# rishikksh20/FastSpeech2

Hardware: NVIDIA H100
Metric: mel-frames/sec (batched inference) (higher is better)
Workload: dtype 3xf16

## Files before the change

fastspeech2_b200/csrc/gemm_tc.cu:

```cuda
#include <stdlib.h>

#include "tc_common.cuh"

namespace fs2 {
namespace {
using namespace tc;

constexpr int BM = 128;
constexpr int BK = 32;
constexpr int A_BYTES = BM * BK * 4;
constexpr int THREADS = 384;
constexpr int PRODUCER_REGS = 40, CONSUMER_REGS = 232;
constexpr int RING_BUDGET = 227 * 1024 - 1024  - 256 ;

struct TcParams {
  int L, tiles_per_utt;
  int m_tiles, n_tiles;
  int B, full, gn, upt, full_tiles;
  int K, taps, pad;
  const float* bias; const float* resid; int ldr; int act;
  float* out; int ldo;
  float a_inv; const float* w_inv;
  __half* outp; __half* outp_lo; int ldo_p;
  float* vt_out; __half* vtp; __half* vtp_lo; int vt_col0, vt_dk, vt_heads, vt_lpad, vt_L;
  const int64_t* lens;
};

template <int BN, bool PRECISE, bool HALF = false>
struct Cfg {
  static constexpr int B_BYTES = BN * BK * 4;
  static constexpr int STAGE_BYTES = (PRECISE ? 2 : 1) * (A_BYTES + B_BYTES);
  static_assert(!PRECISE || HALF, "the error-compensated family is 3xF16");
  static constexpr int STAGES = (RING_BUDGET / STAGE_BYTES) > 8 ? 8 : (RING_BUDGET / STAGE_BYTES);
  static constexpr size_t SMEM = (size_t)STAGES * STAGE_BYTES + 1024 + 256;
  static constexpr int BKE = HALF ? 2 * BK : BK;
  static constexpr int A_LO = A_BYTES;
  static constexpr int B_HI = PRECISE ? 2 * A_BYTES : A_BYTES;
  static constexpr int B_LO = B_HI + B_BYTES;
  static constexpr uint32_t TX_BYTES = (PRECISE ? 2 : 1) * (A_BYTES + B_BYTES);
  static_assert(BN % 16 == 0 && BN >= 16 && BN <= 128, "tile width: sums of wgmma N = 128 / 64 / 16");
  static_assert(B_BYTES % 1024 == 0, "B stage must keep 1024-byte alignment");
  static_assert(STAGES >= 2, "resources");
};

template <int BN, bool HALF, int C0 = 0>
__device__ __forceinline__ void mma_tile(float* d, uint64_t a, uint64_t b, uint32_t acc) {
  if constexpr (BN - C0 >= 128) {
    if constexpr (HALF) wgmma_f16_n128(d + C0 / 2, a, b + (C0 * 128 >> 4), acc); else wgmma_tf32_n128(d + C0 / 2, a, b + (C0 * 128 >> 4), acc);
    mma_tile<BN, HALF, C0 + 128>(d, a, b, acc);
  } else if constexpr (BN - C0 >= 64) {
    if constexpr (HALF) wgmma_f16_n64(d + C0 / 2, a, b + (C0 * 128 >> 4), acc); else wgmma_tf32_n64(d + C0 / 2, a, b + (C0 * 128 >> 4), acc);
    mma_tile<BN, HALF, C0 + 64>(d, a, b, acc);
  } else if constexpr (BN - C0 >= 16) {
    if constexpr (HALF) wgmma_f16_n16(d + C0 / 2, a, b + (C0 * 128 >> 4), acc); else wgmma_tf32_n16(d + C0 / 2, a, b + (C0 * 128 >> 4), acc);
    mma_tile<BN, HALF, C0 + 16>(d, a, b, acc);
  }
}

template <int BN, bool PRECISE, bool HALF>
__global__ void __launch_bounds__(THREADS, 1)
tap_gemm_tc_kernel(const __grid_constant__ CUtensorMap tmap_a, const __grid_constant__ CUtensorMap tmap_b,
                   const __grid_constant__ CUtensorMap tmap_b_lo, const __grid_constant__ CUtensorMap tmap_a16, TcParams p) {
  using C = Cfg<BN, PRECISE, HALF>;
  extern __shared__ uint8_t smem_raw[];
  uint8_t* tiles = smem_raw + ((1024u - (smem_u32(smem_raw) & 1023u)) & 1023u);
  uint64_t* full_bar = reinterpret_cast<uint64_t*>(tiles + (size_t)C::STAGES * C::STAGE_BYTES);
  uint64_t* empty_bar = full_bar + C::STAGES;

  const int warp = uniform_warp_idx(), lane = threadIdx.x & 31;
  const int kchunks = (p.K + C::BKE - 1) / C::BKE;
  const int steps = p.taps * kchunks;
  const int total_tiles = p.m_tiles * p.n_tiles;

  uint64_t* order_bar = empty_bar + C::STAGES;

  if (threadIdx.x == 0) {
    for (int s = 0; s < C::STAGES; ++s) { mbar_init(&full_bar[s], 1); mbar_init(&empty_bar[s], 4); }
    mbar_init(&order_bar[0], 4); mbar_init(&order_bar[1], 4);
    asm volatile("fence.mbarrier_init.release.cluster;" ::: "memory");
  }
  __syncthreads();
  pdl_wait();

  auto tile_coords = [&](int tile, int& n0, int& b, int& t0, int& packed) -> bool {
    const int mt = tile / p.n_tiles;
    n0 = (tile - mt * p.n_tiles) * BN;
    packed = -1;
    if (p.tiles_per_utt == 0) { b = 0; t0 = mt * BM; }
    else if (mt < p.full_tiles) { b = mt / p.full; t0 = (mt - b * p.full) * BM; }
    else { packed = mt - p.full_tiles; b = packed * p.upt; t0 = p.full * BM; }
    return packed < 0 && p.lens != nullptr && t0 >= p.lens[b];
  };

  if (warp < 4) {
    setmaxnreg_dec<PRODUCER_REGS>();
    if (warp != 0) { pdl_trigger(); return; }
    const uint32_t tiles_addr = smem_u32(tiles), full_addr = smem_u32(full_bar);
    int n = 0;
    for (int tile = blockIdx.x; tile < total_tiles; tile += gridDim.x) {
      int n0, b, t0, packed;
      if (tile_coords(tile, n0, b, t0, packed)) continue;
      int j = 0, kc = 0;
      for (int s = 0; s < steps; ++s, ++n) {
        const int slot = n % C::STAGES, round = n / C::STAGES;
        const int k0 = kc * C::BKE, row = t0 + j - p.pad;
        const uint32_t st = tiles_addr + (uint32_t)slot * C::STAGE_BYTES, fb = full_addr + (uint32_t)slot * 8u;
        pin_before(st, fb, k0, row);
        mbar_wait(&empty_bar[slot], (round & 1) ^ 1);
        mbar_expect_tx_elect(fb, C::TX_BYTES);
        if (packed < 0) {
          tma_load_3d_elect(st, &tmap_a, fb, k0, row, b);
          if (PRECISE) tma_load_3d_elect(st + C::A_LO, &tmap_a, fb, k0, row, b + p.B);
        } else {
          for (int g = 0; g < 8; ++g) {
            const int u = g / p.gn, gi = g - u * p.gn;
            const bool real = u < p.upt && b + u < p.B;
            const int oob = PRECISE ? 2 * p.B : p.B;
            tma_load_3d_elect(st + g * (16 * 128), &tmap_a16, fb, k0, row + gi * 16, real ? b + u : oob);
            if (PRECISE) tma_load_3d_elect(st + C::A_LO + g * (16 * 128), &tmap_a16, fb, k0, row + gi * 16, real ? b + u + p.B : oob);
          }
        }
        tma_load_3d_elect(st + C::B_HI, &tmap_b, fb, k0, n0, j);
        if (PRECISE) tma_load_3d_elect(st + C::B_LO, &tmap_b_lo, fb, k0, n0, j);
        if (++kc == kchunks) { kc = 0; ++j; }
      }
    }
  } else {
    setmaxnreg_inc<CONSUMER_REGS>();
    const int cg = (warp >> 2) - 1, wq = warp & 3;
    const int r_lo = 16 * wq + (lane >> 2);
    const int act = p.act, ldr = p.ldr, ldo = p.ldo;
    const float* __restrict__ resid = p.resid; float* __restrict__ out = p.out;
    const bool has_res = resid != nullptr;
    const float oscale = p.a_inv * (p.w_inv ? __ldg(p.w_inv) : 1.0f);
    float d[BN];
    int n = 0;
    int k = 0;
    for (int tile = blockIdx.x; tile < total_tiles; tile += gridDim.x, ++k) {
      int n0, b, t0, packed;
      const int tile_steps = tile_coords(tile, n0, b, t0, packed) ? 0 : steps;
      if ((k & 1) != cg) { n += tile_steps; continue; }
      long m[4]; bool row_ok[4], row_zero[4];
#pragma unroll
      for (int i = 0; i < 4; ++i) {
        const int row = 64 * (i >> 1) + r_lo + 8 * (i & 1);
        int bb = b, t = t0 + row;
        bool ok = t < p.L;
        if (packed >= 0) {
          const int g = row >> 4, u = g / p.gn, gi = g - u * p.gn;
          bb += u;
          t = t0 + gi * 16 + (row & 15);
          ok = u < p.upt && bb < p.B && t < p.L;
        }
        m[i] = (long)bb * p.L + t; row_ok[i] = ok;
        row_zero[i] = ok && p.lens != nullptr && t >= p.lens[bb];
        if (has_res && ok) prefetch_l2(resid + m[i] * ldr + n0);
      }
      if (k > 0) mbar_wait(&order_bar[cg], ((k - 1) >> 1) & 1);
      int prev = -1;
      for (int s = 0; s < tile_steps; ++s, ++n) {
        const int slot = n % C::STAGES, round = n / C::STAGES;
        const uint32_t base = smem_u32(tiles + (size_t)slot * C::STAGE_BYTES);
        const uint64_t a_hi = make_sw128_kmajor_desc(base), b_hi = make_sw128_kmajor_desc(base + C::B_HI);
        const uint64_t a_lo = make_sw128_kmajor_desc(base + C::A_LO), b_lo = make_sw128_kmajor_desc(base + C::B_LO);
        constexpr uint64_t HALF_A = (A_BYTES / 2) >> 4;
        mbar_wait(&full_bar[slot], round & 1);
        wgmma_fence();
#pragma unroll
        for (int kk = 0; kk < 4; ++kk) {
#pragma unroll
          for (int hf = 0; hf < 2; ++hf) {
            float* dh = d + hf * (BN / 2);
            if (PRECISE) {
              mma_tile<BN, true>(dh, a_lo + hf * HALF_A + 2 * kk, b_hi + 2 * kk, (s | kk) != 0);
              mma_tile<BN, true>(dh, a_hi + hf * HALF_A + 2 * kk, b_lo + 2 * kk, 1);
              mma_tile<BN, true>(dh, a_hi + hf * HALF_A + 2 * kk, b_hi + 2 * kk, 1);
            } else {
              mma_tile<BN, HALF>(dh, a_hi + hf * HALF_A + 2 * kk, b_hi + 2 * kk, (s | kk) != 0);
            }
          }
        }
        wgmma_commit();
        wgmma_wait<1>();
        pin_regs<BN>(d);
        if (prev >= 0) { __syncwarp(); if (lane == 0) mbar_arrive(&empty_bar[prev]); }
        prev = slot;
      }
      __syncwarp();
      if (lane == 0) mbar_arrive(&order_bar[cg ^ 1]);
      wgmma_wait<0>();
      pin_regs<BN>(d);
      if (prev >= 0) { __syncwarp(); if (lane == 0) mbar_arrive(&empty_bar[prev]); }
      if (tile_steps == 0) {
#pragma unroll
        for (int i = 0; i < BN; ++i) d[i] = 0.f;
      }

      const bool to_vt = (p.vt_out != nullptr || p.vtp != nullptr) && n0 >= p.vt_col0;
#pragma unroll
      for (int i = 0; i < 4; ++i) {
        if (!row_ok[i] || (to_vt && row_zero[i])) continue;
        const long mm = m[i];
        float* dr = d + (i >> 1) * (BN / 2) + 2 * (i & 1);
#pragma unroll
        for (int jj = 0; jj < BN / 8; ++jj) {
          const int col = n0 + 8 * jj + 2 * (lane & 3);
          float v0 = dr[4 * jj], v1 = dr[4 * jj + 1];
          const float b0 = p.bias ? __ldg(p.bias + col) : 0.f, b1 = p.bias ? __ldg(p.bias + col + 1) : 0.f;
          v0 = fmaf(v0, oscale, b0); v1 = fmaf(v1, oscale, b1);
          if (!to_vt) {
            if (act == ACT_RELU) { v0 = fmaxf(v0, 0.f); v1 = fmaxf(v1, 0.f); }
            else if (act == ACT_TANH) { v0 = tanhf(v0); v1 = tanhf(v1); }
            if (has_res) {
              const float2 r = __ldg(reinterpret_cast<const float2*>(resid + mm * ldr + col));
              v0 += r.x; v1 += r.y;
            }
            if (row_zero[i]) { v0 = 0.f; v1 = 0.f; }
          }
          dr[4 * jj] = v0; dr[4 * jj + 1] = v1;
        }
        if (to_vt) {
          const long ub = mm / p.vt_L;
          const long orow = ub * p.vt_heads * p.vt_dk * (long)p.vt_lpad + (mm - ub * p.vt_L);
#pragma unroll
          for (int jj = 0; jj < BN / 8; ++jj) {
            const int col = n0 + 8 * jj + 2 * (lane & 3);
            const float v0 = dr[4 * jj], v1 = dr[4 * jj + 1];
            const long o = orow + (long)(col - p.vt_col0) * p.vt_lpad;
            if (p.vt_out != nullptr) {
              p.vt_out[o] = v0; p.vt_out[o + p.vt_lpad] = v1;
            } else {
              uint32_t hi, lo;
              split_pair(v0, v1, hi, lo);
              const __half2 h2 = *reinterpret_cast<const __half2*>(&hi), l2 = *reinterpret_cast<const __half2*>(&lo);
              p.vtp[o] = __low2half(h2); p.vtp[o + p.vt_lpad] = __high2half(h2);
              if (p.vtp_lo != nullptr) { p.vtp_lo[o] = __low2half(l2); p.vtp_lo[o + p.vt_lpad] = __high2half(l2); }
            }
          }
          continue;
        }
#pragma unroll
        for (int jj = 0; jj < BN / 8; ++jj) {
          const int col = n0 + 8 * jj + 2 * (lane & 3);
          const float v0 = dr[4 * jj], v1 = dr[4 * jj + 1];
          if (HALF && p.outp != nullptr) {
            const long off = mm * p.ldo_p + col;
            if (p.outp_lo != nullptr) {
              uint32_t hi, lo;
              split_pair(v0, v1, hi, lo);
              *reinterpret_cast<uint32_t*>(p.outp + off) = hi;
              *reinterpret_cast<uint32_t*>(p.outp_lo + off) = lo;
            } else {
              *reinterpret_cast<uint32_t*>(p.outp + off) = hi_pair(v0, v1);
            }
          }
          if (out != nullptr) *reinterpret_cast<float2*>(out + mm * ldo + col) = make_float2(v0, v1);
        }
      }
    }
  }
  pdl_trigger();
}

__global__ void split_rows_f16_kernel(const float* __restrict__ x, int ldx, long rows, int K, __half* __restrict__ S) {
  pdl_trigger(); pdl_wait();
  const int kq = K >> 2;
  const long quads = rows * kq;
  __half* __restrict__ lo_plane = S + rows * K;
  for (long i = (long)blockIdx.x * blockDim.x + threadIdx.x; i < quads; i += (long)gridDim.x * blockDim.x) {
    const long r = i / kq;
    const int c = (int)(i - r * kq) * 4;
    const float4 v = *reinterpret_cast<const float4*>(x + r * ldx + c);
    uint2 hv, lv;
    split_pair(v.x, v.y, hv.x, lv.x);
    split_pair(v.z, v.w, hv.y, lv.y);
    *reinterpret_cast<uint2*>(S + r * K + c) = hv;
    *reinterpret_cast<uint2*>(lo_plane + r * K + c) = lv;
  }
}

template <int BN, bool PRECISE, bool HALF = false>
int launch(const TapGemm& g, cudaStream_t st) {
  using C = Cfg<BN, PRECISE, HALF>;
  static unsigned long long configured = 0;
  int rc;
  if ((rc = ensure_smem_attr(tap_gemm_tc_kernel<BN, PRECISE, HALF>, C::SMEM, &configured))) return rc;
  TcParams p;
  p.K = g.K; p.taps = g.taps; p.pad = (g.taps - 1) / 2;
  p.bias = g.bias; p.resid = g.resid; p.ldr = g.ldr; p.act = g.act; p.out = g.out; p.ldo = g.ldo;
  const long rows = (long)g.B * g.L;
  p.a_inv = HALF ? g.a_inv : 1.0f; p.w_inv = HALF ? g.w_inv : nullptr;
  p.outp = HALF ? g.outp : nullptr; p.ldo_p = g.ldo_p;
  p.outp_lo = (HALF && g.outp && g.outp_lo) ? g.outp + rows * g.ldo_p : nullptr;
  p.vt_out = HALF ? nullptr : g.vt_out; p.vtp = HALF ? g.vtp : nullptr;
  p.vtp_lo = (HALF && g.vtp && g.outp_lo) ? g.vtp + (long)g.B * g.vt_heads * g.vt_dk * g.vt_lpad : nullptr;
  p.vt_col0 = g.vt_col0; p.vt_dk = g.vt_dk; p.vt_heads = g.vt_heads; p.vt_lpad = g.vt_lpad; p.vt_L = g.L;
  p.lens = g.lens;
  CUtensorMap ma, mb, mb_lo, ma16;
  const int esz = HALF ? 2 : 4;
  constexpr int planes = HALF && PRECISE ? 2 : 1;
  const void* xa = HALF ? (const void*)g.xp : (const void*)g.x;
  const uint64_t row_bytes = HALF ? (uint64_t)g.K * 2 : (uint64_t)g.ldx * 4;
  if (g.taps == 1 && g.lens == nullptr) {
    const uint64_t M = (uint64_t)g.B * g.L;
    p.L = (int)M; p.tiles_per_utt = 0;
    p.m_tiles = (int)((M + BM - 1) / BM);
    p.B = 1; p.full = 0; p.gn = 1; p.upt = 1; p.full_tiles = 0;
    if ((rc = make_map(&ma, xa, g.K, M, planes, row_bytes, row_bytes * M, BM, HALF))) return rc;
    ma16 = ma;
  } else {
    p.L = g.L; p.tiles_per_utt = (g.L + BM - 1) / BM;
    p.B = g.B; p.full = g.L / BM;
    int tail = g.L % BM;
    p.gn = tail ? (tail + 15) / 16 : 1;
    p.upt = tail ? 8 / p.gn : 1;
    if (tail && p.upt == 1) { p.full += 1; tail = 0; p.gn = 1; }
    p.full_tiles = p.full * g.B;
    p.m_tiles = p.full_tiles + (tail ? (g.B + p.upt - 1) / p.upt : 0);
    if ((rc = make_map(&ma, xa, g.K, g.L, (uint64_t)g.B * planes, row_bytes, row_bytes * g.L, BM, HALF))) return rc;
    if ((rc = make_map(&ma16, xa, g.K, g.L, (uint64_t)g.B * planes, row_bytes, row_bytes * g.L, 16, HALF))) return rc;
  }
  p.n_tiles = g.N / BN;
  const void* w_hi = HALF ? (const void*)g.w_hi : (const void*)g.w;
  if ((rc = make_map(&mb, w_hi, g.K, g.N, g.taps, (uint64_t)g.K * esz, (uint64_t)g.K * esz * g.N, BN, HALF))) return rc;
  if ((rc = make_map(&mb_lo, PRECISE ? (const void*)g.w_lo : w_hi, g.K, g.N, g.taps, (uint64_t)g.K * esz, (uint64_t)g.K * esz * g.N, BN, HALF))) return rc;
  const int total = p.m_tiles * p.n_tiles;
  const int grid = total < sm_count_current() ? total : sm_count_current();
  FS2_CUDA_CHECK(launch_pdl(tap_gemm_tc_kernel<BN, PRECISE, HALF>, dim3(grid), dim3(THREADS), C::SMEM, st, ma, mb, mb_lo, ma16, p));
  FS2_LAUNCH_CHECK();
  return FS2_OK;
}

int tile_width(int N) { return N % 128 == 0 ? 128 : N % 80 == 0 ? 80 : N % 64 == 0 ? 64 : N % 32 == 0 ? 32 : 16; }

template <bool PRECISE, bool HALF>
int launch_any(const TapGemm& g, cudaStream_t st) {
  switch (tile_width(g.N)) {
    case 128: return launch<128, PRECISE, HALF>(g, st);
    case 80: return launch<80, PRECISE, HALF>(g, st);
    case 64: return launch<64, PRECISE, HALF>(g, st);
    case 32: return launch<32, PRECISE, HALF>(g, st);
    default: return launch<16, PRECISE, HALF>(g, st);
  }
}

int check_output(const TapGemm& g, const char* who) {
  FS2_REQUIRE((g.taps & 1) == 1, "%s: taps must be odd", who);
  FS2_REQUIRE(g.N % 16 == 0, "%s: N (%d) must be a multiple of 16", who, g.N);
  FS2_REQUIRE(!g.resid || g.ldr % 4 == 0, "%s: row strides must be 16-byte multiples", who);
  FS2_REQUIRE(!g.out || (g.ldo % 8 == 0 && (reinterpret_cast<uintptr_t>(g.out) & 31) == 0), "%s: output rows must be 32-byte aligned", who);
  return FS2_OK;
}
int check_common(const TapGemm& g, const char* who) {
  FS2_REQUIRE(g.K % 4 == 0, "%s: K (%d) must be a multiple of 4", who, g.K);
  FS2_REQUIRE(g.ldx % 4 == 0, "%s: row strides must be 16-byte multiples", who);
  FS2_REQUIRE((reinterpret_cast<uintptr_t>(g.x) & 15) == 0 && (reinterpret_cast<uintptr_t>(g.w) & 15) == 0 && g.out != nullptr,
              "%s: operands must be 16-byte aligned", who);
  return check_output(g, who);
}

}

int tap_gemm_tf32(const TapGemm& g, cudaStream_t st) {
  int rc = check_common(g, "tap_gemm_tf32");
  if (rc) return rc;
  FS2_REQUIRE(!g.vt_out || g.vt_col0 % tile_width(g.N) == 0, "tap_gemm_tf32: the transposed V third must start at a tile boundary");
  if ((long)g.B * g.L == 0) return FS2_OK;
  return launch_any<false, false>(g, st);
}

int tap_gemm_planes(const TapGemm& g, cudaStream_t st) {
  const char* who = g.precise ? "tap_gemm_planes(3xF16)" : "tap_gemm_planes(f16)";
  FS2_REQUIRE(g.xp && g.w_hi && (!g.precise || g.w_lo) && (g.out || g.outp || g.vtp), "%s: operand planes / an output missing", who);
  FS2_REQUIRE(g.K % 8 == 0, "%s: K (%d) must be a multiple of 8 (16-byte plane rows)", who, g.K);
  FS2_REQUIRE((reinterpret_cast<uintptr_t>(g.xp) & 15) == 0 && (reinterpret_cast<uintptr_t>(g.w_hi) & 15) == 0, "%s: operands must be 16-byte aligned", who);
  FS2_REQUIRE(!g.outp || (g.ldo_p % 16 == 0 && (reinterpret_cast<uintptr_t>(g.outp) & 31) == 0 && (((long)g.B * g.L * g.ldo_p) % 16) == 0),
              "%s: output plane rows must be 32-byte aligned", who);
  {
    const int bn = tile_width(g.N);
    FS2_REQUIRE(!g.vtp || (g.vt_lpad % 8 == 0 && g.N % bn == 0 && g.vt_col0 % bn == 0 && g.vt_dk % 32 == 0),
                "%s: transposed V planes need a 16-byte row pitch and tile-aligned thirds", who);
  }
  int rc = check_output(g, who);
  if (rc) return rc;
  if ((long)g.B * g.L == 0) return FS2_OK;
  return g.precise ? launch_any<true, true>(g, st) : launch_any<false, true>(g, st);
}

int split_rows(const float* x, int ldx, long rows, int K, __half* planes, cudaStream_t st) {
  if (rows == 0) return FS2_OK;
  FS2_REQUIRE(K % 4 == 0 && ldx % 4 == 0, "split_rows: K and the row stride must be multiples of 4");
  const long quads = rows * (K / 4);
  long blocks = (quads + 255) / 256;
  FS2_CUDA_CHECK(launch_pdl(split_rows_f16_kernel, dim3((unsigned)(blocks > 132 * 16 ? 132 * 16 : blocks)), dim3(256), 0, st, x, ldx, rows, K, planes));
  FS2_LAUNCH_CHECK();
  return FS2_OK;
}

namespace {
__global__ void split_f16_kernel(const float* __restrict__ src, __half* __restrict__ hi, __half* __restrict__ lo, long n,
                                 const float* __restrict__ scale) {
  const float s = scale ? __ldg(scale) : 1.0f;
  for (long i = (long)blockIdx.x * blockDim.x + threadIdx.x; i < n; i += (long)gridDim.x * blockDim.x) {
    const float x = fminf(fmaxf(src[i] * s, -65504.f), 65504.f);
    const __half h = __float2half_rn(x);
    hi[i] = h; lo[i] = __float2half_rn(x - __half2float(h));
  }
}
__global__ void weight_scale_kernel(const float* __restrict__ w, long n, float* __restrict__ scale, float* __restrict__ inv) {
  __shared__ float red[32];
  float m = 0.f;
  for (long i = threadIdx.x; i < n; i += blockDim.x) m = fmaxf(m, fabsf(w[i]));
  m = warp_max(m);
  if ((threadIdx.x & 31) == 0) red[threadIdx.x >> 5] = m;
  __syncthreads();
  if (threadIdx.x < 32) {
    m = threadIdx.x < (blockDim.x >> 5) ? red[threadIdx.x] : 0.f;
    m = warp_max(m);
    if (threadIdx.x == 0) {
      int k = 0;
      if (m > 0.f && isfinite(m)) {
        int e;
        frexpf(m, &e);
        k = 14 - e;
        k = k > 60 ? 60 : (k < -60 ? -60 : k);
      }
      scale[0] = ldexpf(1.0f, k); inv[0] = ldexpf(1.0f, -k);
    }
  }
}
}

namespace {
__global__ void planes_to_rows_kernel(const __half* __restrict__ planes, long n, float* __restrict__ out) {
  for (long i = (long)blockIdx.x * blockDim.x + threadIdx.x; i < n; i += (long)gridDim.x * blockDim.x)
    out[i] = (__half2float(planes[i]) + __half2float(planes[n + i])) * kPlaneInv;
}
}

int planes_to_rows(const __half* planes, long n, float* out, cudaStream_t st) {
  if (n == 0) return FS2_OK;
  long blocks = (n + 255) / 256;
  planes_to_rows_kernel<<<(int)(blocks > 1184 ? 1184 : blocks), 256, 0, st>>>(planes, n, out);
  FS2_LAUNCH_CHECK();
  return FS2_OK;
}

int split_f16(const float* src, __half* hi, __half* lo, long n, const float* scale, cudaStream_t st) {
  if (n == 0) return FS2_OK;
  long blocks = (n + 255) / 256;
  split_f16_kernel<<<(int)(blocks > 1184 ? 1184 : blocks), 256, 0, st>>>(src, hi, lo, n, scale);
  FS2_LAUNCH_CHECK();
  return FS2_OK;
}

int weight_scale(const float* w, long n, float* scale, float* inv, cudaStream_t st) {
  weight_scale_kernel<<<1, 1024, 0, st>>>(w, n, scale, inv);
  FS2_LAUNCH_CHECK();
  return FS2_OK;
}

}
```

Baseline: 2.927 million.

## Load conv halo A tile once per k-chunk and reuse across taps

Splits the shared-memory ring into separate A and B rings. For multi-tap convolutions the A tile is loaded once per k-chunk as a halo box of BM+taps-1 rows and reused across all taps by shifting the descriptor base by one row per tap; previously each tap reloaded a full A tile. Ring depths are computed at launch time and the loop order becomes k-chunk outer, taps inner. This cuts A-operand TMA traffic by roughly the tap count, at the cost of more complex barrier bookkeeping. The one-row descriptor offset relies on the swizzle layout lining up, which is a correctness risk.

```diff
diff --git a/fastspeech2_b200/csrc/gemm_tc.cu b/fastspeech2_b200/csrc/gemm_tc.cu
--- a/fastspeech2_b200/csrc/gemm_tc.cu
+++ b/fastspeech2_b200/csrc/gemm_tc.cu
@@ -11,13 +11,18 @@
 constexpr int A_BYTES = BM * BK * 4;
 constexpr int THREADS = 384;
 constexpr int PRODUCER_REGS = 40, CONSUMER_REGS = 232;
-constexpr int RING_BUDGET = 227 * 1024 - 1024  - 256 ;
+constexpr int MAX_DEPTH = 8;
+constexpr int BAR_BYTES = (4 * MAX_DEPTH + 2) * 8;
+constexpr int SMEM_MAX = 227 * 1024;
+constexpr int RING_BUDGET = SMEM_MAX - 1024  - BAR_BYTES;
+constexpr int MAX_BOX_ROWS = 256;
 
 struct TcParams {
   int L, tiles_per_utt;
   int m_tiles, n_tiles;
   int B, full, gn, upt, full_tiles;
   int K, taps, pad;
+  int a_rows, a_plane, a_slot, a_depth, b_depth;
   const float* bias; const float* resid; int ldr; int act;
   float* out; int ldo;
   float a_inv; const float* w_inv;
@@ -28,20 +33,30 @@
 
 template <int BN, bool PRECISE, bool HALF = false>
 struct Cfg {
+  static constexpr int PLANES = PRECISE ? 2 : 1;
   static constexpr int B_BYTES = BN * BK * 4;
-  static constexpr int STAGE_BYTES = (PRECISE ? 2 : 1) * (A_BYTES + B_BYTES);
+  static constexpr int B_SLOT = PLANES * B_BYTES;
   static_assert(!PRECISE || HALF, "the error-compensated family is 3xF16");
-  static constexpr int STAGES = (RING_BUDGET / STAGE_BYTES) > 8 ? 8 : (RING_BUDGET / STAGE_BYTES);
-  static constexpr size_t SMEM = (size_t)STAGES * STAGE_BYTES + 1024 + 256;
   static constexpr int BKE = HALF ? 2 * BK : BK;
-  static constexpr int A_LO = A_BYTES;
-  static constexpr int B_HI = PRECISE ? 2 * A_BYTES : A_BYTES;
-  static constexpr int B_LO = B_HI + B_BYTES;
-  static constexpr uint32_t TX_BYTES = (PRECISE ? 2 : 1) * (A_BYTES + B_BYTES);
   static_assert(BN % 16 == 0 && BN >= 16 && BN <= 128, "tile width: sums of wgmma N = 128 / 64 / 16");
-  static_assert(B_BYTES % 1024 == 0, "B stage must keep 1024-byte alignment");
-  static_assert(STAGES >= 2, "resources");
+  static_assert(B_BYTES % 1024 == 0, "B slot must keep 1024-byte alignment");
 };
+
+template <int BN, bool PRECISE, bool HALF>
+bool ring_layout(int taps, TcParams& p) {
+  using C = Cfg<BN, PRECISE, HALF>;
+  p.a_rows = BM + taps - 1;
+  p.a_plane = (p.a_rows * 128 + 1023) / 1024 * 1024;
+  p.a_slot = C::PLANES * p.a_plane;
+  auto cap = [](int d) { return d > MAX_DEPTH ? MAX_DEPTH : d; };
+  if (taps == 1) {
+    p.a_depth = p.b_depth = cap(RING_BUDGET / (p.a_slot + C::B_SLOT));
+  } else {
+    p.b_depth = cap((RING_BUDGET - 2 * p.a_slot) / C::B_SLOT);
+    p.a_depth = cap((RING_BUDGET - p.b_depth * C::B_SLOT) / p.a_slot);
+  }
+  return p.a_rows <= MAX_BOX_ROWS && p.a_depth >= 2 && p.b_depth >= 2;
+}
 
 template <int BN, bool HALF, int C0 = 0>
 __device__ __forceinline__ void mma_tile(float* d, uint64_t a, uint64_t b, uint32_t acc) {
@@ -64,18 +79,23 @@
   using C = Cfg<BN, PRECISE, HALF>;
   extern __shared__ uint8_t smem_raw[];
   uint8_t* tiles = smem_raw + ((1024u - (smem_u32(smem_raw) & 1023u)) & 1023u);
-  uint64_t* full_bar = reinterpret_cast<uint64_t*>(tiles + (size_t)C::STAGES * C::STAGE_BYTES);
-  uint64_t* empty_bar = full_bar + C::STAGES;
+  uint8_t* b_ring = tiles + (size_t)p.a_depth * p.a_slot;
+  uint64_t* full_a = reinterpret_cast<uint64_t*>(b_ring + (size_t)p.b_depth * C::B_SLOT);
+  uint64_t* empty_a = full_a + MAX_DEPTH;
+  uint64_t* full_b = empty_a + MAX_DEPTH;
+  uint64_t* empty_b = full_b + MAX_DEPTH;
+  uint64_t* order_bar = empty_b + MAX_DEPTH;
 
   const int warp = uniform_warp_idx(), lane = threadIdx.x & 31;
+  const int taps = p.taps, a_depth = p.a_depth, b_depth = p.b_depth;
+  const bool joint = taps == 1;
   const int kchunks = (p.K + C::BKE - 1) / C::BKE;
-  const int steps = p.taps * kchunks;
+  const int steps = taps * kchunks;
   const int total_tiles = p.m_tiles * p.n_tiles;
 
-  uint64_t* order_bar = empty_bar + C::STAGES;
-
   if (threadIdx.x == 0) {
-    for (int s = 0; s < C::STAGES; ++s) { mbar_init(&full_bar[s], 1); mbar_init(&empty_bar[s], 4); }
+    for (int s = 0; s < a_depth; ++s) { mbar_init(&full_a[s], 1); mbar_init(&empty_a[s], 4); }
+    for (int s = 0; s < b_depth; ++s) { mbar_init(&full_b[s], 1); mbar_init(&empty_b[s], 4); }
     mbar_init(&order_bar[0], 4); mbar_init(&order_bar[1], 4);
     asm volatile("fence.mbarrier_init.release.cluster;" ::: "memory");
   }
@@ -95,34 +115,54 @@
   if (warp < 4) {
     setmaxnreg_dec<PRODUCER_REGS>();
     if (warp != 0) { pdl_trigger(); return; }
-    const uint32_t tiles_addr = smem_u32(tiles), full_addr = smem_u32(full_bar);
-    int n = 0;
+    const uint32_t a_addr = smem_u32(tiles), b_addr = smem_u32(b_ring);
+    const uint32_t full_a_addr = smem_u32(full_a), full_b_addr = smem_u32(full_b);
+    const uint32_t a_tx = (uint32_t)(C::PLANES * p.a_rows * 128), packed_tx = (uint32_t)(C::PLANES * A_BYTES);
+    int sa = 0, pa = 0, sb = 0, pb = 0;
     for (int tile = blockIdx.x; tile < total_tiles; tile += gridDim.x) {
       int n0, b, t0, packed;
       if (tile_coords(tile, n0, b, t0, packed)) continue;
-      int j = 0, kc = 0;
-      for (int s = 0; s < steps; ++s, ++n) {
-        const int slot = n % C::STAGES, round = n / C::STAGES;
-        const int k0 = kc * C::BKE, row = t0 + j - p.pad;
-        const uint32_t st = tiles_addr + (uint32_t)slot * C::STAGE_BYTES, fb = full_addr + (uint32_t)slot * 8u;
-        pin_before(st, fb, k0, row);
-        mbar_wait(&empty_bar[slot], (round & 1) ^ 1);
-        mbar_expect_tx_elect(fb, C::TX_BYTES);
-        if (packed < 0) {
-          tma_load_3d_elect(st, &tmap_a, fb, k0, row, b);
-          if (PRECISE) tma_load_3d_elect(st + C::A_LO, &tmap_a, fb, k0, row, b + p.B);
-        } else {
-          for (int g = 0; g < 8; ++g) {
-            const int u = g / p.gn, gi = g - u * p.gn;
-            const bool real = u < p.upt && b + u < p.B;
-            const int oob = PRECISE ? 2 * p.B : p.B;
-            tma_load_3d_elect(st + g * (16 * 128), &tmap_a16, fb, k0, row + gi * 16, real ? b + u : oob);
-            if (PRECISE) tma_load_3d_elect(st + C::A_LO + g * (16 * 128), &tmap_a16, fb, k0, row + gi * 16, real ? b + u + p.B : oob);
+      const int row0 = t0 - p.pad;
+      const uint32_t a_bytes = packed < 0 ? a_tx : packed_tx;
+      for (int kc = 0; kc < kchunks; ++kc) {
+        const int k0 = kc * C::BKE;
+        for (int j = 0; j < taps; ++j) {
+          const uint32_t stb = b_addr + (uint32_t)(sb * C::B_SLOT), fbb = full_b_addr + (uint32_t)sb * 8u;
+          if (packed >= 0 || j == 0) {
+            const uint32_t st = a_addr + (uint32_t)(sa * p.a_slot);
+            const uint32_t fb = joint ? fbb : full_a_addr + (uint32_t)sa * 8u;
+            const int row = packed < 0 ? row0 : row0 + j;
+            pin_before(st, fb, k0, row);
+            if (joint) {
+              mbar_wait(&empty_b[sb], pb ^ 1);
+              mbar_expect_tx_elect(fb, a_bytes + C::B_SLOT);
+            } else {
+              mbar_wait(&empty_a[sa], pa ^ 1);
+              mbar_expect_tx_elect(fb, a_bytes);
+            }
+            if (packed < 0) {
+              tma_load_3d_elect(st, &tmap_a, fb, k0, row, b);
+              if (PRECISE) tma_load_3d_elect(st + p.a_plane, &tmap_a, fb, k0, row, b + p.B);
+            } else {
+              for (int g = 0; g < 8; ++g) {
+                const int u = g / p.gn, gi = g - u * p.gn;
+                const bool real = u < p.upt && b + u < p.B;
+                const int oob = PRECISE ? 2 * p.B : p.B;
+                tma_load_3d_elect(st + g * (16 * 128), &tmap_a16, fb, k0, row + gi * 16, real ? b + u : oob);
+                if (PRECISE) tma_load_3d_elect(st + p.a_plane + g * (16 * 128), &tmap_a16, fb, k0, row + gi * 16, real ? b + u + p.B : oob);
+              }
+            }
+            if (++sa == a_depth) { sa = 0; pa ^= 1; }
           }
-        }
-        tma_load_3d_elect(st + C::B_HI, &tmap_b, fb, k0, n0, j);
-        if (PRECISE) tma_load_3d_elect(st + C::B_LO, &tmap_b_lo, fb, k0, n0, j);
-        if (++kc == kchunks) { kc = 0; ++j; }
+          if (!joint) {
+            pin_before(stb, fbb, k0, j);
+            mbar_wait(&empty_b[sb], pb ^ 1);
+            mbar_expect_tx_elect(fbb, C::B_SLOT);
+          }
+          tma_load_3d_elect(stb, &tmap_b, fbb, k0, n0, j);
+          if (PRECISE) tma_load_3d_elect(stb + C::B_BYTES, &tmap_b_lo, fbb, k0, n0, j);
+          if (++sb == b_depth) { sb = 0; pb ^= 1; }
+        }
       }
     }
   } else {
@@ -134,12 +174,17 @@
     const bool has_res = resid != nullptr;
     const float oscale = p.a_inv * (p.w_inv ? __ldg(p.w_inv) : 1.0f);
     float d[BN];
-    int n = 0;
+    int sa = 0, pa = 0, sb = 0, pb = 0;
+    auto skip = [](int& slot, int& phase, int n, int depth) { slot += n; phase ^= (slot / depth) & 1; slot %= depth; };
     int k = 0;
     for (int tile = blockIdx.x; tile < total_tiles; tile += gridDim.x, ++k) {
       int n0, b, t0, packed;
       const int tile_steps = tile_coords(tile, n0, b, t0, packed) ? 0 : steps;
-      if ((k & 1) != cg) { n += tile_steps; continue; }
+      if ((k & 1) != cg) {
+        skip(sa, pa, tile_steps == 0 ? 0 : packed < 0 ? kchunks : steps, a_depth);
+        skip(sb, pb, tile_steps, b_depth);
+        continue;
+      }
       long m[4]; bool row_ok[4], row_zero[4];
 #pragma unroll
       for (int i = 0; i < 4; ++i) {
@@ -157,14 +202,22 @@
         if (has_res && ok) prefetch_l2(resid + m[i] * ldr + n0);
       }
       if (k > 0) mbar_wait(&order_bar[cg], ((k - 1) >> 1) & 1);
-      int prev = -1;
-      for (int s = 0; s < tile_steps; ++s, ++n) {
-        const int slot = n % C::STAGES, round = n / C::STAGES;
-        const uint32_t base = smem_u32(tiles + (size_t)slot * C::STAGE_BYTES);
-        const uint64_t a_hi = make_sw128_kmajor_desc(base), b_hi = make_sw128_kmajor_desc(base + C::B_HI);
-        const uint64_t a_lo = make_sw128_kmajor_desc(base + C::A_LO), b_lo = make_sw128_kmajor_desc(base + C::B_LO);
+      int prev_b = -1, prev_a = -1;
+      int slot_a = 0, j = 0;
+      for (int s = 0; s < tile_steps; ++s) {
+        if (packed >= 0 || j == 0) {
+          slot_a = sa;
+          if (!joint) mbar_wait(&full_a[sa], pa);
+          if (++sa == a_depth) { sa = 0; pa ^= 1; }
+        }
+        const int slot_b = sb, phase_b = pb;
+        if (++sb == b_depth) { sb = 0; pb ^= 1; }
+        const uint32_t a_base = smem_u32(tiles + (size_t)slot_a * p.a_slot) + (packed < 0 ? (uint32_t)j * 128u : 0u);
+        const uint32_t b_base = smem_u32(b_ring + (size_t)slot_b * C::B_SLOT);
+        const uint64_t a_hi = make_sw128_kmajor_desc(a_base), b_hi = make_sw128_kmajor_desc(b_base);
+        const uint64_t a_lo = make_sw128_kmajor_desc(a_base + p.a_plane), b_lo = make_sw128_kmajor_desc(b_base + C::B_BYTES);
         constexpr uint64_t HALF_A = (A_BYTES / 2) >> 4;
-        mbar_wait(&full_bar[slot], round & 1);
+        mbar_wait(&full_b[slot_b], phase_b);
         wgmma_fence();
 #pragma unroll
         for (int kk = 0; kk < 4; ++kk) {
@@ -183,14 +236,22 @@
         wgmma_commit();
         wgmma_wait<1>();
         pin_regs<BN>(d);
-        if (prev >= 0) { __syncwarp(); if (lane == 0) mbar_arrive(&empty_bar[prev]); }
-        prev = slot;
+        if (prev_b >= 0) {
+          __syncwarp();
+          if (lane == 0) { mbar_arrive(&empty_b[prev_b]); if (!joint && prev_a >= 0) mbar_arrive(&empty_a[prev_a]); }
+        }
+        prev_b = slot_b;
+        prev_a = packed >= 0 || j == taps - 1 ? slot_a : -1;
+        if (++j == taps) j = 0;
       }
       __syncwarp();
       if (lane == 0) mbar_arrive(&order_bar[cg ^ 1]);
       wgmma_wait<0>();
       pin_regs<BN>(d);
-      if (prev >= 0) { __syncwarp(); if (lane == 0) mbar_arrive(&empty_bar[prev]); }
+      if (prev_b >= 0) {
+        __syncwarp();
+        if (lane == 0) { mbar_arrive(&empty_b[prev_b]); if (!joint && prev_a >= 0) mbar_arrive(&empty_a[prev_a]); }
+      }
       if (tile_steps == 0) {
 #pragma unroll
         for (int i = 0; i < BN; ++i) d[i] = 0.f;
@@ -282,10 +343,13 @@
 template <int BN, bool PRECISE, bool HALF = false>
 int launch(const TapGemm& g, cudaStream_t st) {
   using C = Cfg<BN, PRECISE, HALF>;
+  TcParams p;
+  FS2_REQUIRE((ring_layout<BN, PRECISE, HALF>(g.taps, p)), "tap GEMM: taps = %d: a halo box of %d rows exceeds the TMA box limit (%d rows) or the shared-memory rings",
+              g.taps, BM + g.taps - 1, MAX_BOX_ROWS);
+  const size_t smem = (size_t)p.a_depth * p.a_slot + (size_t)p.b_depth * C::B_SLOT + 1024 + BAR_BYTES;
   static unsigned long long configured = 0;
   int rc;
-  if ((rc = ensure_smem_attr(tap_gemm_tc_kernel<BN, PRECISE, HALF>, C::SMEM, &configured))) return rc;
-  TcParams p;
+  if ((rc = ensure_smem_attr(tap_gemm_tc_kernel<BN, PRECISE, HALF>, SMEM_MAX, &configured))) return rc;
   p.K = g.K; p.taps = g.taps; p.pad = (g.taps - 1) / 2;
   p.bias = g.bias; p.resid = g.resid; p.ldr = g.ldr; p.act = g.act; p.out = g.out; p.ldo = g.ldo;
   const long rows = (long)g.B * g.L;
@@ -317,7 +381,7 @@
     if (tail && p.upt == 1) { p.full += 1; tail = 0; p.gn = 1; }
     p.full_tiles = p.full * g.B;
     p.m_tiles = p.full_tiles + (tail ? (g.B + p.upt - 1) / p.upt : 0);
-    if ((rc = make_map(&ma, xa, g.K, g.L, (uint64_t)g.B * planes, row_bytes, row_bytes * g.L, BM, HALF))) return rc;
+    if ((rc = make_map(&ma, xa, g.K, g.L, (uint64_t)g.B * planes, row_bytes, row_bytes * g.L, p.a_rows, HALF))) return rc;
     if ((rc = make_map(&ma16, xa, g.K, g.L, (uint64_t)g.B * planes, row_bytes, row_bytes * g.L, 16, HALF))) return rc;
   }
   p.n_tiles = g.N / BN;
@@ -326,7 +390,7 @@
   if ((rc = make_map(&mb_lo, PRECISE ? (const void*)g.w_lo : w_hi, g.K, g.N, g.taps, (uint64_t)g.K * esz, (uint64_t)g.K * esz * g.N, BN, HALF))) return rc;
   const int total = p.m_tiles * p.n_tiles;
   const int grid = total < sm_count_current() ? total : sm_count_current();
-  FS2_CUDA_CHECK(launch_pdl(tap_gemm_tc_kernel<BN, PRECISE, HALF>, dim3(grid), dim3(THREADS), C::SMEM, st, ma, mb, mb_lo, ma16, p));
+  FS2_CUDA_CHECK(launch_pdl(tap_gemm_tc_kernel<BN, PRECISE, HALF>, dim3(grid), dim3(THREADS), smem, st, ma, mb, mb_lo, ma16, p));
   FS2_LAUNCH_CHECK();
   return FS2_OK;
 }
```

Result: slower. 2.874 million, median of 6 (-1.8%).
